# bexcite/ptudes-lab

Hardware: AMD Instinct MI355X
Metric: lidar scans/sec (ICP+EKF) on 128x1024 sweeps (higher is better)
Workload: dtype f64

## Files before the change

### ptudes-lab_amd/csrc/icp_kernels.h

```cpp
#pragma once
#include "devmath.h"
#include "diag.h"
#include <stdint.h>
#include <type_traits>

#define EMPTY_KEY 0xFFFFFFFFFFFFFFFFull
#define TOMB_KEY 0xFFFFFFFFFFFFFFFEull
#define KEY_OFF (1 << 20)

#define ERR_KEY_RANGE 1
#define ERR_POOL 2
#define ERR_TABLE 4
#define ERR_VDS_TABLE 8
#define ERR_GN_TIMEOUT 16

struct TabEnt {
    unsigned long long key;
    int blk;
    int head;
};
#define BLK_ID_MASK 0x00FFFFFF

struct VdsEnt {
    unsigned long long key;
    unsigned vmin;
    unsigned pad;
};
struct ScanStats {
    double sigma, err_dt, err_drot;
    int iterations, n_corr_last;
    long long n_in, n_valid, n_down, n_src, sum_cand, map_voxels, map_points;
};

struct DevState {
    int n_in, n_valid, n_down, n_src;
    unsigned gn_epoch;
    int gn_iters, gn_ncorr;
    int gn_abort;
    int dbg_dead_wg;
    long long gn_cand;
    double gn_max_dist, gn_kernel;
    double T_icp[16];
    double lin_sums[32];
    long long gn_phase_clk[8];
    long long seq_clk[8];
    int n_poses, has_ext_guess;
    double pose_first[16], pose_prev[16], pose_last[16];
    double guess[16], new_pose[16];
    double xi[6];
    int do_deskew, pad1;
    double sigma, sse;
    long long n_samples;
    double model_dev[16];
    int prev_n_in, pending_finish;
    int pro_next;
    int n_src_last;
    int n_down_ins;
    int stats_pending;
    int pool_hw, pool_hw_s;
    int free_top, n_live;
    int free_top_s, mig_n;
    int ulist_n, ulist_pad;
    long long map_points;
    unsigned tab_used;
    int err_flags;
    unsigned long long exec_cnt[8];
    unsigned long long sched_cnt[4];
    unsigned long long empty_cnt;
    unsigned long long full_cnt;
    const double* dk_knots;
    const long long* dk_nknots;
    const int* dk_kovf;
    const double* dk_t0t1;
    int* dk_modes;
    int dk_n, dk_pad;
};
#define DK_MODE_NONE 0
#define DK_MODE_CV 1
#define DK_MODE_IMU 2

struct Ctx {
    double max_range, min_range, vs, vds1, vds2, init_thr, min_motion, conv;
    int P, deskew, max_iter, W;
    const float* in_f32;
    const double* in_f64;
// ... 207 lines not shown
            Rt d = rt_mul(rt_inv(rt_from16(sp[0])), rt_from16(sp[2]));
            moved = sqrt(d.t[0] * d.t[0] + d.t[1] * d.t[1] + d.t[2] * d.t[2]) > 5.0 * c.min_motion;
        }
        s_moved = moved ? 1 : 0;
    }
    if (threadIdx.x == 128) {
        Rt dev = rt_from16(sp[4]);
        const double theta = rot_angle(dev.R);
        s_err = sqrt(dev.t[0] * dev.t[0] + dev.t[1] * dev.t[1] + dev.t[2] * dev.t[2]) + 2.0 * c.max_range * sin(0.5 * theta);
    }
    if (threadIdx.x == 192 && !c.ext_guess) {
        Rt last = rt_from16(sp[2]);
        Rt pred = (n_poses >= 2) ? rt_mul(rt_inv(rt_from16(sp[1])), last) : rt_identity();
        Rt lp = (n_poses >= 1) ? last : rt_identity();
        rt_to16(rt_mul(lp, pred), st->guess);
    }
    __syncthreads();
    if (threadIdx.x == 0) {
        double sigma = c.init_thr;
        if (s_moved) {
            const double err = s_err;
            if (err > c.min_motion) { st->sse += err * err; st->n_samples += 1; }
            sigma = (st->n_samples < 1) ? c.init_thr : sqrt(st->sse / (double)st->n_samples);
        }
        st->sigma = sigma;
        st->gn_max_dist = 3.0 * sigma;
        st->gn_kernel = sigma / 3.0;
    }
    __threadfence_block();
    if (s_closed && threadIdx.x < 48) {
        const int a = threadIdx.x >> 4, k = threadIdx.x & 15;
        double* dst = a == 0 ? st->pose_first : a == 1 ? st->pose_prev : st->pose_last;
        if (a > 0 || s_closed == 2) dst[k] = sp[a][k];
    }
    __syncthreads();
    gn_ll_clear_on_wrap(c);
    if (IMU && st->dk_knots) {
        d_imu_coltab(st, c.coltab, c.W, (c.deskew && c.t01 == nullptr) ? 1 : 0, n_poses);
        return;
    }
    if (st->do_deskew && c.t01 == nullptr) {
        double xi[6];
        for (int k = 0; k < 6; ++k) xi[k] = st->xi[k];
        for (int j = threadIdx.x; j < c.W; j += blockDim.x) {
            const double sft = (double)j * (1.0 / (double)c.W) - 0.5;
            double x[6];
            for (int k = 0; k < 6; ++k) x[k] = sft * xi[k];
            const Rt M = se3_exp(x);
            double* o = c.coltab + (size_t)j;
            for (int k = 0; k < 9; ++k) o[(size_t)k * c.W] = M.R[k];
            for (int k = 0; k < 3; ++k) o[(size_t)(9 + k) * c.W] = M.t[k];
        }
    }
}

__global__ __launch_bounds__(256) void k_build_lut(int H, int W, const double* alt_deg, const double* az_deg, double n_mm,
                                                   const double* T16_mm, double* dir_out, double* off_out) {
    const int i = blockIdx.x * 256 + threadIdx.x;
    if (i >= H * W) return;
    const int u = i / W, v = i % W;
    const double kPi = 3.14159265358979323846;
    const double enc = 2.0 * kPi * (1.0 - (double)v / (double)W);
    const double az = -az_deg[u] * kPi / 180.0, phi = alt_deg[u] * kPi / 180.0;
    const double dx = cos(enc + az) * cos(phi), dy = sin(enc + az) * cos(phi), dz = sin(phi);
    const double ox = n_mm * (cos(enc) - dx), oy = n_mm * (sin(enc) - dy), oz = -n_mm * dz;
    const double* T = T16_mm;
    for (int r = 0; r < 3; ++r) {
        dir_out[3 * (size_t)i + r] = (T[4 * r] * dx + T[4 * r + 1] * dy + T[4 * r + 2] * dz) * 1e-3;
        off_out[3 * (size_t)i + r] = (T[4 * r] * ox + T[4 * r + 1] * oy + T[4 * r + 2] * oz + T[4 * r + 3]) * 1e-3;
    }
}

struct Slice { int b, nb, clk; };
__device__ __forceinline__ Slice launch_slice() { Slice s; s.b = (int)blockIdx.x; s.nb = (int)gridDim.x; s.clk = 0; return s; }
#define STAGE_MAX_WAVES 16
#define STAGE_MAX_U 16

struct VdsPass {
    int* slot;
    VdsEnt* tab;
    unsigned mask;
    int* bcnt;
    const double* in;
    double* out;
    int DevState::*n_out;
    int n;
    DevState* st;
};
__device__ __forceinline__ VdsPass vds_pass1(const Ctx& c) { return VdsPass{c.slot1, c.vtab1, c.vmask, c.bcnt1, c.pts, c.fd, &DevState::n_down, c.n_in, c.st}; }
__device__ __forceinline__ VdsPass vds_pass2(const Ctx& c) { return VdsPass{c.slot2, c.vtab2, c.vmask2, c.bcnt2, c.fd, c.src0, &DevState::n_src, c.st->n_down, c.st}; }

template <int U>
__device__ __forceinline__ void vds_claim_u(VdsEnt* tab, unsigned mask, const unsigned long long (&key)[U], const bool (&want)[U],
                                            int (&slot)[U]) {
    unsigned sp[U];
    unsigned long long old[U];
    bool pend[U];
#pragma unroll
    for (int u = 0; u < U; ++u) {
        sp[u] = brick_slot(key[u], mask);
        slot[u] = -1;
        old[u] = key[u];
        if (want[u]) old[u] = atomicCAS(&tab[sp[u]].key, EMPTY_KEY, key[u]);
    }
#pragma unroll
    for (int u = 0; u < U; ++u) {
        pend[u] = want[u] && !(old[u] == EMPTY_KEY || old[u] == key[u]);
        if (want[u] && !pend[u]) slot[u] = (int)sp[u];
    }
    for (unsigned probe = 1; probe <= mask; ++probe) {
        bool anyp = false;
#pragma unroll
        for (int u = 0; u < U; ++u) anyp = anyp || pend[u];
        if (!anyp) break;
#pragma unroll
        for (int u = 0; u < U; ++u)
            if (pend[u]) { sp[u] = (sp[u] + 1) & mask; old[u] = atomicCAS(&tab[sp[u]].key, EMPTY_KEY, key[u]); }
#pragma unroll
        for (int u = 0; u < U; ++u)
            if (pend[u] && (old[u] == EMPTY_KEY || old[u] == key[u])) { slot[u] = (int)sp[u]; pend[u] = false; }
    }
}
template <int U>
__device__ __forceinline__ void vds_bid_u(VdsEnt* tab, const int (&slot)[U], const bool (&want)[U], const int (&idx)[U], int* err_flags) {
#pragma unroll
    for (int u = 0; u < U; ++u) {
        if (!want[u]) continue;
        if (slot[u] < 0) atomicOr(err_flags, ERR_VDS_TABLE);
        else atomicMin(&tab[slot[u]].vmin, (unsigned)idx[u]);
    }
}
struct VdsNoLap { __device__ __forceinline__ void operator()() const {} };
template <int U, class Between = VdsNoLap>
__device__ __forceinline__ void vds_claim_run_heads(VdsEnt* tab, unsigned mask, const unsigned long long (&key)[U], const bool (&has_key)[U],
                                                    const int (&idx)[U], int (&slot_out)[U], unsigned long long* exec_counter, int* err_flags,
                                                    Between between = Between()) {
    const int lane = threadIdx.x & 63;
    bool head[U];
    int slot[U];
#pragma unroll
    for (int u = 0; u < U; ++u) {
        const unsigned long long prev = __shfl_up(key[u], 1);
        const bool prev_has_key = __shfl_up(has_key[u] ? 1 : 0, 1) != 0;
        head[u] = has_key[u] && (lane == 0 || !prev_has_key || prev != key[u]);
    }
    vds_claim_u<U>(tab, mask, key, head, slot);
    {
        int nh = 0;
#pragma unroll
        for (int u = 0; u < U; ++u) nh += __popcll(__ballot(head[u]));
        if (lane == 0 && nh) atomicAdd(exec_counter, (unsigned long long)nh);
    }
    between();
    vds_bid_u<U>(tab, slot, head, idx, err_flags);
#pragma unroll
    for (int u = 0; u < U; ++u) slot_out[u] = head[u] ? slot[u] : -1;
}
template <int U>
__device__ __forceinline__ int block_count_u(const bool (&f)[U]) {
    __shared__ int cnt[STAGE_MAX_WAVES];
    int mine = 0;
#pragma unroll
    for (int u = 0; u < U; ++u) mine += __popcll(__ballot(f[u]));
    if ((threadIdx.x & 63) == 0) cnt[threadIdx.x >> 6] = mine;
    __syncthreads();
    int tot = 0;
    for (int k = 0; k < ((int)blockDim.x >> 6); ++k) tot += cnt[k];
    __syncthreads();
    return tot;
}

template <int U> struct RawF32 { float v[U][3]; };
template <int U>
__device__ __forceinline__ RawF32<U> k1_load_raw(const Ctx& c, const Slice sl) {
    RawF32<U> r;
    const int BS = (int)blockDim.x, base = sl.b * BS * U + (int)threadIdx.x;
#pragma unroll
    for (int u = 0; u < U; ++u) {
        const int i = base + u * BS;
        const bool in = i < c.n_in;
        r.v[u][0] = in ? c.in_f32[3 * (size_t)i] : 0.0f; r.v[u][1] = in ? c.in_f32[3 * (size_t)i + 1] : 0.0f; r.v[u][2] = in ? c.in_f32[3 * (size_t)i + 2] : 0.0f;
    }
    return r;
}
template <int U>
__device__ __forceinline__ void d_deskew_vds1(const Ctx& c, const Slice sl, const RawF32<U>* pre = nullptr, int* wave_valid = nullptr) {
    const int BS = (int)blockDim.x, base = sl.b * BS * U + (int)threadIdx.x;
    DevState* st = c.st;
    DiagLap<diag::stages, false, true> k1(sl.clk != 0 && threadIdx.x == 0);
    const int do_deskew = st->do_deskew;
    int idx[U];
    bool valid[U], keyed[U];
    unsigned long long key[U];
    V3 p[U];
#pragma unroll
    for (int u = 0; u < U; ++u) idx[u] = base + u * BS;
    k1.lap(c, D_k1_entry);
#pragma unroll
    for (int u = 0; u < U; ++u) {
        const int i = idx[u];
        p[u] = v3(0.0, 0.0, 0.0);
        if (i < c.n_in) {
            if (c.in_range) {
                unsigned rg = c.in_range[i];
                if (c.row_mask && !c.row_mask[i / c.W]) rg = 0;
                const double r = (double)rg;
                const double* d = c.lut_dir + 3 * (size_t)i;
                const double* o = c.lut_off + 3 * (size_t)i;
                p[u] = rg ? v3(r * d[0] + o[0], r * d[1] + o[1], r * d[2] + o[2]) : v3(0.0, 0.0, 0.0);
            } else if (c.in_f32) {
                if (pre) p[u] = v3((double)pre->v[u][0], (double)pre->v[u][1], (double)pre->v[u][2]);
                else p[u] = v3((double)c.in_f32[3 * (size_t)i], (double)c.in_f32[3 * (size_t)i + 1], (double)c.in_f32[3 * (size_t)i + 2]);
            } else {
                p[u] = v3(c.in_f64[3 * (size_t)i], c.in_f64[3 * (size_t)i + 1], c.in_f64[3 * (size_t)i + 2]);
            }
        }
    }
    Rt Mcol[2];
    const bool col_period2 = U > 2 && ((2 * BS) % c.W) == 0;
#pragma unroll
    for (int u = 0; u < U; ++u) {
        const int i = idx[u];
        valid[u] = false; keyed[u] = false; key[u] = EMPTY_KEY;
        if (i < c.n_in) {
            if (do_deskew) {
                if (c.t01) {
                    const double s = c.t01[i] - 0.5;
                    double x[6];
                    for (int k = 0; k < 6; ++k) x[k] = s * st->xi[k];
                    p[u] = rt_apply(se3_exp(x), p[u]);
                } else {
                    Rt& M = (u & 1) ? Mcol[1] : Mcol[0];
                    if (u < 2 || !col_period2) {
                        const double* m = c.coltab + (size_t)(i % c.W);
                        for (int k = 0; k < 9; ++k) M.R[k] = m[(size_t)k * c.W];
                        for (int k = 0; k < 3; ++k) M.t[k] = m[(size_t)(9 + k) * c.W];
                    }
                    p[u] = rt_apply(M, p[u]);
                }
            }
            const double r = sqrt(p[u].x * p[u].x + p[u].y * p[u].y + p[u].z * p[u].z);
            valid[u] = (r < c.max_range) && (r > c.min_range);
            if (valid[u]) {
                c.pts[3 * (size_t)i] = p[u].x; c.pts[3 * (size_t)i + 1] = p[u].y; c.pts[3 * (size_t)i + 2] = p[u].z;
                int kx, ky, kz;
                keyed[u] = vox_key(p[u], c.vds1, key[u], kx, ky, kz);
                if (!keyed[u]) atomicOr(&st->err_flags, ERR_KEY_RANGE);
            }
        }
    }
    k1.lap(c, D_k1_load_deskew_store);
    {
        const VdsPass p1 = vds_pass1(c);
        int slot[U];
        vds_claim_run_heads<U>(p1.tab, p1.mask, key, keyed, idx, slot, &st->exec_cnt[4], &st->err_flags, [&] { k1.lap(c, D_k1_claim); });
        k1.lap(c, D_k1_bid);
#pragma unroll
        for (int u = 0; u < U; ++u)
            if (idx[u] < p1.n) p1.slot[idx[u]] = slot[u];
    }
    k1.lap(c, D_k1_slot1);
    if (wave_valid) {
        int nvw = 0;
#pragma unroll
        for (int u = 0; u < U; ++u) nvw += __popcll(__ballot(valid[u]));
        *wave_valid += nvw;
    } else {
        const int nv = block_count_u<U>(valid);
        if (threadIdx.x == 0 && nv) atomicAdd(&st->n_valid, nv);
    }
    k1.lap(c, D_k1_count);
}

template <int U> struct PreI32 { int v[U]; };
template <int U>
__device__ __forceinline__ PreI32<U> stage_load_i32(const int* arr, int n, const Slice sl) {
    PreI32<U> r;
    const int BS = (int)blockDim.x, base = sl.b * BS * U + (int)threadIdx.x;
#pragma unroll
    for (int u = 0; u < U; ++u) { const int i = base + u * BS; r.v[u] = (i < n) ? arr[i] : -1; }
    return r;
}

__device__ __forceinline__ int block_offset_part(const int* bcnt, int b) {
    int s = 0;
    for (int k = threadIdx.x; k < b; k += (int)blockDim.x) s += bcnt[k];
    return s;
}
__device__ __forceinline__ int block_offset(int s) {
    __shared__ int red[STAGE_MAX_WAVES];
    const int nw = (int)blockDim.x >> 6;
    for (int o = 32; o > 0; o >>= 1) s += __shfl_down(s, o);
    if ((threadIdx.x & 63) == 0) red[threadIdx.x >> 6] = s;
    __syncthreads();
    int tot = 0;
    for (int k = 0; k < nw; ++k) tot += red[k];
    __syncthreads();
    return tot;
}
template <int U>
__device__ __forceinline__ void block_rank_u(const bool (&f)[U], int (&rk)[U], int& total) {
    __shared__ int red[STAGE_MAX_U][STAGE_MAX_WAVES];
    const int lane = threadIdx.x & 63, wv = threadIdx.x >> 6, nw = (int)blockDim.x >> 6;
    int within[U];
#pragma unroll
    for (int u = 0; u < U; ++u) {
        const unsigned long long m = __ballot(f[u]);
        within[u] = __popcll(m & ((1ull << lane) - 1ull));
        if (lane == 0) red[u][wv] = __popcll(m);
    }
    __syncthreads();
    int running = 0;
#pragma unroll
    for (int u = 0; u < U; ++u) {
        int off = 0, tot = 0;
        for (int k = 0; k < nw; ++k) { const int v = red[u][k]; if (k < wv) off += v; tot += v; }
        rk[u] = running + off + within[u];
        running += tot;
    }
    total = running;
    __syncthreads();
}
#define LOOKBACK_POLLS (1u << 22)
__device__ __forceinline__ void lookback_publish(int* bcnt, int b, unsigned tag, int count) {
    if (threadIdx.x == 0) __hip_atomic_store(&bcnt[b], (int)((tag << 16) | (unsigned)count), __ATOMIC_RELAXED, __HIP_MEMORY_SCOPE_AGENT);
}
__device__ __forceinline__ int lookback_offset(const int* bcnt, int b, unsigned tag, DevState* st) {
    int s = 0;
    bool bad = false;
    for (int k = threadIdx.x; k < b; k += (int)blockDim.x) {
        unsigned polls = 0;
        for (;;) {
            const unsigned v = (unsigned)__hip_atomic_load(&bcnt[k], __ATOMIC_RELAXED, __HIP_MEMORY_SCOPE_AGENT);
            if ((v >> 16) == tag) { s += (int)(v & 0xFFFFu); break; }
            if (++polls > LOOKBACK_POLLS || ((polls & 1023u) == 0u && __hip_atomic_load(&st->gn_abort, __ATOMIC_RELAXED, __HIP_MEMORY_SCOPE_AGENT) != 0)) { bad = true; break; }
            __builtin_amdgcn_s_sleep(1);
        }
    }
    if (bad) { atomicOr(&st->err_flags, ERR_GN_TIMEOUT); __hip_atomic_store(&st->gn_abort, 1, __ATOMIC_RELAXED, __HIP_MEMORY_SCOPE_AGENT); }
    return block_offset(s);
}
__device__ __forceinline__ unsigned lookback_tag(int scan_k) { return ((unsigned)scan_k % 0xFFFFu) + 1u; }
static_assert(STAGE_MAX_U * 1024 < (1 << 16), "the look-back word keeps a block's count in 16 bits");

template <int U>
__device__ __forceinline__ void d_count_winners(const VdsPass& p, const Slice sl) {
    const int BS = (int)blockDim.x, base = sl.b * BS * U + (int)threadIdx.x;
    int idx[U], s[U];
    bool w[U];
#pragma unroll
    for (int u = 0; u < U; ++u) { idx[u] = base + u * BS; s[u] = (idx[u] < p.n) ? p.slot[idx[u]] : -1; }
    {
        unsigned vm[U];
#pragma unroll
        for (int u = 0; u < U; ++u) vm[u] = (s[u] >= 0) ? p.tab[s[u]].vmin : 0u;
#pragma unroll
        for (int u = 0; u < U; ++u) w[u] = (s[u] >= 0) && (vm[u] == (unsigned)idx[u]);
    }
    const int nw = block_count_u<U>(w);
    if (threadIdx.x == 0) p.bcnt[sl.b] = nw;
}

template <int U, bool LB>
__device__ __forceinline__ void d_compact_winners(const VdsPass& p, const Slice sl, const PreI32<U>* pre = nullptr, unsigned tag = 0u) {
    const int BS = (int)blockDim.x, base = sl.b * BS * U + (int)threadIdx.x;
    int idx[U], s[U], rk[U];
    bool w[U];
    int off_part = 0;
    if (!LB) off_part = block_offset_part(p.bcnt, sl.b);
#pragma unroll
    for (int u = 0; u < U; ++u) { idx[u] = base + u * BS; s[u] = pre ? pre->v[u] : ((idx[u] < p.n) ? p.slot[idx[u]] : -1); }
    {
        unsigned vm[U];
#pragma unroll
        for (int u = 0; u < U; ++u) vm[u] = (s[u] >= 0) ? p.tab[s[u]].vmin : 0u;
#pragma unroll
        for (int u = 0; u < U; ++u) w[u] = (s[u] >= 0) && (vm[u] == (unsigned)idx[u]);
    }
    double q[U][3];
#pragma unroll
    for (int u = 0; u < U; ++u) {
        const size_t i = (size_t)idx[u];
        if (w[u]) { q[u][0] = p.in[3 * i]; q[u][1] = p.in[3 * i + 1]; q[u][2] = p.in[3 * i + 2]; }
    }
    int total;
    block_rank_u<U>(w, rk, total);
    int off;
    if (LB) {
        lookback_publish(p.bcnt, sl.b, tag, total);
        off = lookback_offset(p.bcnt, sl.b, tag, p.st);
    } else {
        off = block_offset(off_part);
    }
#pragma unroll
    for (int u = 0; u < U; ++u) {
        if (!w[u]) continue;
        const size_t o = (size_t)(off + rk[u]) * 3;
        p.out[o] = q[u][0]; p.out[o + 1] = q[u][1]; p.out[o + 2] = q[u][2];
        p.tab[s[u]].key = EMPTY_KEY;
        p.tab[s[u]].vmin = 0xFFFFFFFFu;
    }
    if (threadIdx.x == 0 && sl.b == sl.nb - 1) p.st->*p.n_out = off + total;
}

template <int U>
__device__ __forceinline__ void d_vds2_fd(const Ctx& c, const Slice sl) {
    const int BS = (int)blockDim.x, base = sl.b * BS * U + (int)threadIdx.x;
    const VdsPass p2 = vds_pass2(c);
    int idx[U];
    bool act[U];
    unsigned long long key[U];
#pragma unroll
    for (int u = 0; u < U; ++u) { idx[u] = base + u * BS; act[u] = idx[u] < p2.n; key[u] = EMPTY_KEY; }
    {
        double q[U][3];
#pragma unroll
        for (int u = 0; u < U; ++u) {
            const size_t j = (size_t)idx[u];
            q[u][0] = q[u][1] = q[u][2] = 0.0;
            if (act[u]) { q[u][0] = p2.in[3 * j]; q[u][1] = p2.in[3 * j + 1]; q[u][2] = p2.in[3 * j + 2]; }
        }
#pragma unroll
        for (int u = 0; u < U; ++u) {
            if (!act[u]) continue;
            int kx, ky, kz;
            vox_key(v3(q[u][0], q[u][1], q[u][2]), c.vds2, key[u], kx, ky, kz);
        }
    }
    int slot[U];
    vds_claim_run_heads<U>(p2.tab, p2.mask, key, act, idx, slot, &c.st->exec_cnt[5], &c.st->err_flags);
#pragma unroll
    for (int u = 0; u < U; ++u)
        if (act[u]) p2.slot[idx[u]] = slot[u];
}

template <class CT>
__device__ __forceinline__ int map_find(const CT& c, unsigned long long key) {
    unsigned s = brick_slot(key, c.tmask);
    for (unsigned probe = 0; probe <= c.tmask; ++probe) {
        const TabEnt e = c.tab[s];
        if (e.key == key) return e.blk;
        if (e.key == EMPTY_KEY) return -1;
        s = (s + 1) & c.tmask;
    }
    return -1;
}

__device__ __forceinline__ double sqrt_gate(double M) {
    if (!(M > 0.0) || !(M < 1.0e150)) return (M > 0.0) ? M : 0.0;
    double T = M * M;
    for (int k = 0; k < 64 && sqrt(__longlong_as_double(__double_as_longlong(T) - 1)) >= M; ++k)
        T = __longlong_as_double(__double_as_longlong(T) - 1);
    for (int k = 0; k < 64 && sqrt(T) < M; ++k) T = __longlong_as_double(__double_as_longlong(T) + 1);
    return T;
}

template <int CTRL>
__device__ __forceinline__ double dpp_f64(double v) {
    const unsigned long long u = (unsigned long long)__double_as_longlong(v);
    const unsigned lo = (unsigned)__builtin_amdgcn_update_dpp(0, (int)(unsigned)u, CTRL, 0xF, 0xF, true);
    const unsigned hi = (unsigned)__builtin_amdgcn_update_dpp(0, (int)(unsigned)(u >> 32), CTRL, 0xF, 0xF, true);
    return __longlong_as_double((long long)(((unsigned long long)hi << 32) | lo));
}
__device__ __forceinline__ double group_min32(double v) {
    v = fmin(v, dpp_f64<0xB1>(v));
    v = fmin(v, dpp_f64<0x4E>(v));
    v = fmin(v, dpp_f64<0x141>(v));
    v = fmin(v, dpp_f64<0x140>(v));
    return fmin(v, __shfl_xor(v, 16));
}
__device__ __forceinline__ unsigned group_min32(unsigned v) {
    v = min(v, (unsigned)__builtin_amdgcn_update_dpp(0, (int)v, 0xB1, 0xF, 0xF, true));
    v = min(v, (unsigned)__builtin_amdgcn_update_dpp(0, (int)v, 0x4E, 0xF, 0xF, true));
    v = min(v, (unsigned)__builtin_amdgcn_update_dpp(0, (int)v, 0x141, 0xF, 0xF, true));
    v = min(v, (unsigned)__builtin_amdgcn_update_dpp(0, (int)v, 0x140, 0xF, 0xF, true));
    return min(v, (unsigned)__shfl_xor((int)v, 16));
}

__device__ __forceinline__ int group_sum32(int v) {
    v += __builtin_amdgcn_update_dpp(0, v, 0xB1, 0xF, 0xF, true);
    v += __builtin_amdgcn_update_dpp(0, v, 0x4E, 0xF, 0xF, true);
    v += __builtin_amdgcn_update_dpp(0, v, 0x141, 0xF, 0xF, true);
    v += __builtin_amdgcn_update_dpp(0, v, 0x140, 0xF, 0xF, true);
// ... 1751 lines not shown
    const int cnt = blk_hdr(c, b)[0];
    if (cnt <= 0) return;
    const int o = atomicAdd(counter, cnt);
    const double* X = blk_x(c, b);
    for (int j = 0; j < cnt; ++j) {
        if (o + j >= max_points) break;
        out[3 * (size_t)(o + j)] = X[3 * j]; out[3 * (size_t)(o + j) + 1] = X[3 * j + 1]; out[3 * (size_t)(o + j) + 2] = X[3 * j + 2];
    }
}

__global__ __launch_bounds__(256) void k_deskew_only(Ctx c, const double* xyz, const double* t01, int n, double* out) {
    const int i = blockIdx.x * 256 + threadIdx.x;
    if (i >= n) return;
    const DevState* st = c.st;
    V3 p = v3(xyz[3 * (size_t)i], xyz[3 * (size_t)i + 1], xyz[3 * (size_t)i + 2]);
    if (c.deskew && st->n_poses >= 2) {
        double xi[6], x[6];
        se3_log(rt_mul(rt_inv(rt_from16(st->pose_prev)), rt_from16(st->pose_last)), xi);
        const double sft = t01[i] - 0.5;
        for (int k = 0; k < 6; ++k) x[k] = sft * xi[k];
        p = rt_apply(se3_exp(x), p);
    }
    out[3 * (size_t)i] = p.x; out[3 * (size_t)i + 1] = p.y; out[3 * (size_t)i + 2] = p.z;
}

__global__ __launch_bounds__(1024) void k_range_stats(const unsigned* range, int H, int W, const unsigned char* row_mask,
                                                      double to_m, double* out) {
    __shared__ double sh[1024];
    __shared__ double shmin[1024], shmax[1024];
    __shared__ double s_mean, s_n;
    const int tid = threadIdx.x, n_all = H * W;
    for (int pass = 0; pass < 2; ++pass) {
        const double mean = pass ? s_mean : 0.0;
        double acc = 0.0, cnt = 0.0, lo = 1.7976931348623157e308, hi = -1.7976931348623157e308;
        for (int i = tid; i < n_all; i += 1024) {
            const unsigned r = range[i];
            if (r == 0 || (row_mask && !row_mask[i / W])) continue;
            const double x = (double)r * to_m;
            if (pass == 0) { acc += x; cnt += 1.0; lo = fmin(lo, x); hi = fmax(hi, x); }
            else { const double d = x - mean; acc += d * d; }
        }
        sh[tid] = acc;
        __syncthreads();
        for (int o = 512; o > 0; o >>= 1) { if (tid < o) sh[tid] += sh[tid + o]; __syncthreads(); }
        const double total = sh[0];
        __syncthreads();
        if (pass == 0) {
            sh[tid] = cnt; shmin[tid] = lo; shmax[tid] = hi;
            __syncthreads();
            for (int o = 512; o > 0; o >>= 1) {
                if (tid < o) { sh[tid] += sh[tid + o]; shmin[tid] = fmin(shmin[tid], shmin[tid + o]); shmax[tid] = fmax(shmax[tid], shmax[tid + o]); }
                __syncthreads();
            }
            if (tid == 0) {
                s_n = sh[0];
                s_mean = sh[0] > 0.0 ? total / sh[0] : 0.0;
                out[0] = sh[0]; out[1] = s_mean; out[3] = shmin[0]; out[4] = shmax[0];
            }
            __syncthreads();
        } else if (tid == 0) {
            out[2] = s_n > 0.0 ? total / s_n : 0.0;
        }
    }
}

struct EkfState;
struct SeqCtx {
    Ctx c;
    const float* scan_base;
    long long scan_stride_floats;
    int input_is_range, n_scans;
    double* fd_buf[2];
    EkfState* ekf;
    const double* imu;
    const int* imu_end;
    double *res_poses, *res_t, *rows;
};
__device__ __forceinline__ Ctx load_seq_ctx(const SeqCtx* a, int s, int scan_k) {
    Ctx c = a[s].c;
    c.fd = a[s].fd_buf[scan_k & 1];
    const float* p = a[s].scan_base + (size_t)scan_k * (size_t)a[s].scan_stride_floats;
    if (a[s].input_is_range) { c.in_range = (const unsigned*)p; c.in_f32 = nullptr; }
    else { c.in_f32 = p; c.in_range = nullptr; }
    c.in_f32 = uniform_ptr(c.in_f32); c.in_range = uniform_ptr(c.in_range);
    c.pts = uniform_ptr(c.pts);
    c.slot1 = uniform_ptr(c.slot1); c.vtab1 = uniform_ptr(c.vtab1); c.bcnt1 = uniform_ptr(c.bcnt1);
    c.slot2 = uniform_ptr(c.slot2); c.vtab2 = uniform_ptr(c.vtab2); c.bcnt2 = uniform_ptr(c.bcnt2);
    c.fd = uniform_ptr(c.fd); c.fdw = uniform_ptr(c.fdw); c.src0 = uniform_ptr(c.src0); c.coltab = uniform_ptr(c.coltab);
    c.pslot = uniform_ptr(c.pslot); c.nxt = uniform_ptr(c.nxt); c.prank = uniform_ptr(c.prank); c.plen = uniform_ptr(c.plen);
    c.tab = uniform_ptr(c.tab); c.blocks = uniform_ptr(c.blocks); c.free_stack = uniform_ptr(c.free_stack); c.st = uniform_ptr(c.st);
    c.bhdr = uniform_ptr(c.bhdr); c.bfirst = uniform_ptr(c.bfirst); c.big_base = uniform_ptr(c.big_base);
    c.free_stack_s = uniform_ptr(c.free_stack_s); c.mig_list = uniform_ptr(c.mig_list);
    return c;
}
__global__ __launch_bounds__(1024) void k_scan_prologue(Ctx c) { d_scan_prologue<false>(c); }
__global__ __launch_bounds__(1024) void k_scan_prologue_imu(Ctx c) { d_scan_prologue<true>(c); }
__global__ __launch_bounds__(1024) void kb_scan_prologue(const SeqCtx* a, int scan_k) {
    const Ctx c = load_seq_ctx(a, blockIdx.y, scan_k);
    d_scan_prologue<false>(c);
}
__global__ __launch_bounds__(1024) void kb_scan_prologue_imu(const SeqCtx* a, int scan_k) {
    const Ctx c = load_seq_ctx(a, blockIdx.y, scan_k);
    d_scan_prologue<true>(c);
}
__global__ __launch_bounds__(256) void k_deskew_vds1(Ctx c) { d_deskew_vds1<1>(c, launch_slice()); }
__global__ __launch_bounds__(256) void kb_deskew_vds1(const SeqCtx* a, int scan_k) {
    const Ctx c = load_seq_ctx(a, blockIdx.y, scan_k);
    d_deskew_vds1<1>(c, launch_slice());
}
__global__ __launch_bounds__(256) void k_count_w1(Ctx c) { d_count_winners<1>(vds_pass1(c), launch_slice()); }
__global__ __launch_bounds__(256) void kb_count_w1(const SeqCtx* a, int scan_k) {
    const Ctx c = load_seq_ctx(a, blockIdx.y, scan_k);
    d_count_winners<1>(vds_pass1(c), launch_slice());
}
__global__ __launch_bounds__(256) void k_compact_fd(Ctx c) { d_compact_winners<1, false>(vds_pass1(c), launch_slice()); }
__global__ __launch_bounds__(256) void kb_compact_fd(const SeqCtx* a, int scan_k) {
    const Ctx c = load_seq_ctx(a, blockIdx.y, scan_k);
    d_compact_winners<1, false>(vds_pass1(c), launch_slice());
}
__global__ __launch_bounds__(256) void k_vds2_fd(Ctx c) { d_vds2_fd<1>(c, launch_slice()); }
__global__ __launch_bounds__(256) void kb_vds2_fd(const SeqCtx* a, int scan_k) {
    const Ctx c = load_seq_ctx(a, blockIdx.y, scan_k);
    d_vds2_fd<1>(c, launch_slice());
}
__global__ __launch_bounds__(256) void k_count_w2(Ctx c) { d_count_winners<1>(vds_pass2(c), launch_slice()); }
__global__ __launch_bounds__(256) void kb_count_w2(const SeqCtx* a, int scan_k) {
    const Ctx c = load_seq_ctx(a, blockIdx.y, scan_k);
    d_count_winners<1>(vds_pass2(c), launch_slice());
}
__global__ __launch_bounds__(256) void k_compact_src(Ctx c) { d_compact_winners<1, false>(vds_pass2(c), launch_slice()); }
__global__ __launch_bounds__(256) void kb_compact_src(const SeqCtx* a, int scan_k) {
    const Ctx c = load_seq_ctx(a, blockIdx.y, scan_k);
    d_compact_winners<1, false>(vds_pass2(c), launch_slice());
}
__global__ __launch_bounds__(256) void k_map_insert_a(Ctx c, const double* pts_in, const int* n_ptr, int n_fixed, int use_pose) { d_map_insert_a<1>(c, pts_in, n_ptr, n_fixed, use_pose, launch_slice()); }
__global__ __launch_bounds__(256) void kb_map_insert_a(const SeqCtx* a, int scan_k) {
    const Ctx c = load_seq_ctx(a, blockIdx.y, scan_k);
    d_map_insert_a<1>(c, c.fd, &c.st->n_down_ins, 0, 1, launch_slice());
}
__global__ __launch_bounds__(256) void k_map_insert_b(Ctx c, const int* n_ptr, int n_fixed) { d_map_insert_b<1>(c, n_ptr, n_fixed, launch_slice()); }
__global__ __launch_bounds__(256) void kb_map_insert_b(const SeqCtx* a, int scan_k) {
    const Ctx c = load_seq_ctx(a, blockIdx.y, scan_k);
    d_map_insert_b<1>(c, &c.st->n_down_ins, 0, launch_slice());
}
__global__ __launch_bounds__(256) void k_map_insert_c(Ctx c, const int* n_ptr, int n_fixed) { d_map_insert_c<1>(c, n_ptr, n_fixed, launch_slice()); }
__global__ __launch_bounds__(256) void kb_map_insert_c(const SeqCtx* a, int scan_k) {
    const Ctx c = load_seq_ctx(a, blockIdx.y, scan_k);
    d_map_insert_c<1>(c, &c.st->n_down_ins, 0, launch_slice());
}
__global__ __launch_bounds__(256) void k_map_prune(Ctx c, const double* origin_xyz, int use_new_pose) { d_map_prune<1>(c, origin_xyz, use_new_pose, launch_slice()); }
__global__ __launch_bounds__(256) void kb_map_prune(const SeqCtx* a, int scan_k) {
    const Ctx c = load_seq_ctx(a, blockIdx.y, scan_k);
    d_map_prune<1>(c, nullptr, 1, launch_slice());
}
__global__ __launch_bounds__(256) void k_map_rebuild(Ctx c) { d_map_rebuild(c, launch_slice()); }
__global__ __launch_bounds__(256) void kb_map_rebuild(const SeqCtx* a, int scan_k) {
    const Ctx c = load_seq_ctx(a, blockIdx.y, scan_k);
    d_map_rebuild(c, launch_slice());
}

#define GN_MAX_SEQ 256
__device__ __forceinline__ bool kx_assign(int S, int& s, int& G, int& wg) {
    const int x = (int)(blockIdx.x & 7u), j = (int)(blockIdx.x >> 3), J = (int)(gridDim.x >> 3);
    const int spx = S <= 8 ? 1 : (S <= 16 ? 2 : 4);
    G = J / spx;
    s = x + 8 * (j / G);
    wg = j % G;
    return s < S;
}
template <int PC, int GC>
__global__ __launch_bounds__(GN8_MAX_THREADS) SEQ_OCC void kx_gn_loop8(const SeqCtx* a, int S, int scan_k) {
    int s, G, wg;
    if (!kx_assign(S, s, G, wg)) return;
    const Ctx c = load_seq_ctx(a, s, scan_k);
    gn8_body<PC, GC>(c, 0, G, wg);
}
template <int PC>
__global__ __launch_bounds__(GN_MAX_THREADS) void kx_gn_loop(const SeqCtx* a, int S, int scan_k) {
    int s, G, wg;
    if (!kx_assign(S, s, G, wg)) return;
    const Ctx c = load_seq_ctx(a, s, scan_k);
    gn_loop_body<PC, true, true>(c, 0, G, wg);
}
```

### ptudes-lab_amd/csrc/seq_kernel.h

```cpp
#pragma once
#include "ekf_kernels.h"
#include "icp_kernels.h"

#define TEAM_BAR_POLLS (1u << 23)
__device__ __forceinline__ bool team_sync(unsigned* word, unsigned n, unsigned& target, int* abort_word, DevState* st, const bool local) {
    __shared__ int s_bad;
    if (n <= 1u) {
        asm volatile("s_waitcnt vmcnt(0)" ::: "memory");
        __syncthreads();
        __builtin_amdgcn_fence(__ATOMIC_ACQUIRE, "agent");
        return true;
    }
    if (local) asm volatile("s_waitcnt vmcnt(0)" ::: "memory");
    __syncthreads();
    target += n;
    if (threadIdx.x == 0) {
        int bad = 0;
        if (!local) __builtin_amdgcn_fence(__ATOMIC_RELEASE, "agent");
        __hip_atomic_fetch_add(word, 1u, __ATOMIC_RELAXED, __HIP_MEMORY_SCOPE_AGENT);
        unsigned polls = 0;
        while (__hip_atomic_load(word, __ATOMIC_RELAXED, __HIP_MEMORY_SCOPE_AGENT) < target) {
            __builtin_amdgcn_s_sleep(2);
            if ((++polls & 255u) == 0u && (gn_abort_seen(abort_word) || polls > TEAM_BAR_POLLS)) { bad = 1; break; }
        }
        if (bad) {
            if (st) gn_raise_abort(st);
            __hip_atomic_store(abort_word, 1, __ATOMIC_RELAXED, __HIP_MEMORY_SCOPE_AGENT);
        }
        s_bad = bad;
    }
    __syncthreads();
    __builtin_amdgcn_fence(__ATOMIC_ACQUIRE, "agent");
    return s_bad == 0;
}
struct TeamEnv { unsigned* word; int* abort_word; DevState* st; bool local; };
__device__ __forceinline__ bool team_sync(const TeamEnv& e, unsigned n, unsigned& target) { return team_sync(e.word, n, target, e.abort_word, e.st, e.local); }
__device__ __forceinline__ unsigned xcc_id() {
    unsigned v;
    asm volatile("s_getreg_b32 %0, hwreg(HW_REG_XCC_ID)" : "=s"(v));
    return v & 0xFu;
}

#define SEQ_FAIL 0xFFFFFFFFu
#ifndef SEQ_U
#define SEQ_U 8
#endif
#ifndef SEQ_UM
#define SEQ_UM SEQ_U
#endif
#ifndef SEQ_UM_ALT
#define SEQ_UM_ALT 4
#endif
#ifndef SEQ_U2
#define SEQ_U2 16
#endif
__device__ __noinline__ void sq_prologue(const SeqCtx* a, int s, int k) { d_scan_prologue(load_seq_ctx(a, s, k), true); }
__device__ __noinline__ unsigned sq_prepare(const SeqCtx* a, int s, int k, int wg, int nw, unsigned target, unsigned* word, bool local) {
    const Ctx c = load_seq_ctx(a, s, k);
    DevState* st = c.st;
    const int BS = (int)blockDim.x * SEQ_U, nbs = (c.n_in + BS - 1) / BS;
    const int BS2 = (int)blockDim.x * SEQ_U2, nbs2 = (c.n_in + BS2 - 1) / BS2;
    Slice sl;
    sl.nb = nbs; sl.clk = wg == 0 ? 1 : 0;
    const TeamEnv te = {word, &st->gn_abort, st, local};
    DiagLap<diag::stages, false, false> sq(wg == 0 && threadIdx.x == 0);
    if (wg == 0 && st->pro_next != k + 1) sq_prologue(a, s, k);
    sq.lap(c, D_sq_prologue);
    if (!team_sync(te, (unsigned)nw, target)) return SEQ_FAIL;
    sq.lap(c, D_sq_wait_prologue);
    int wave_valid = 0;
    if (c.in_f32 && !c.in_range) {
        RawF32<SEQ_U> raw;
        sl.b = wg;
        if (wg < nbs) raw = k1_load_raw<SEQ_U>(c, sl);
        for (sl.b = wg; sl.b < nbs; sl.b += nw) {
            const RawF32<SEQ_U> cur = raw;
            Slice nx = sl;
            nx.b = sl.b + nw;
            if (nx.b < nbs) raw = k1_load_raw<SEQ_U>(c, nx);
            d_deskew_vds1<SEQ_U>(c, sl, &cur, &wave_valid);
        }
    } else {
        for (sl.b = wg; sl.b < nbs; sl.b += nw) d_deskew_vds1<SEQ_U>(c, sl, nullptr, &wave_valid);
    }
    if ((threadIdx.x & 63) == 0 && wave_valid) atomicAdd(&st->n_valid, wave_valid);
    sq.lap(c, D_sq_deskew_vds1);
    if (!team_sync(te, (unsigned)nw, target)) return SEQ_FAIL;
    sq.lap(c, D_sq_wait_deskew_vds1);
    sl.nb = nbs2;
    const unsigned tag = lookback_tag(k);
    {
        PreI32<SEQ_U2> pw;
        sl.b = wg;
        if (wg < nbs2) pw = stage_load_i32<SEQ_U2>(c.slot1, c.n_in, sl);
        for (sl.b = wg; sl.b < nbs2; sl.b += nw) {
            const PreI32<SEQ_U2> cur = pw;
            Slice nx = sl;
            nx.b = sl.b + nw;
            if (nx.b < nbs2) pw = stage_load_i32<SEQ_U2>(c.slot1, c.n_in, nx);
            d_compact_winners<SEQ_U2, true>(vds_pass1(c), sl, &cur, tag);
        }
    }
    sq.lap(c, D_sq_compact_fd);
    if (!team_sync(te, (unsigned)nw, target)) return SEQ_FAIL;
    sq.lap(c, D_sq_wait_compact_fd);
    const int nbf = (st->n_down + BS2 - 1) / BS2;
    sl.nb = nbf;
    for (sl.b = wg; sl.b < nbf; sl.b += nw) d_vds2_fd<SEQ_U2>(c, sl);
    sq.lap(c, D_sq_vds2);
    if (!team_sync(te, (unsigned)nw, target)) return SEQ_FAIL;
    sq.lap(c, D_sq_wait_vds2);
    for (sl.b = wg; sl.b < nbf; sl.b += nw) d_compact_winners<SEQ_U2, true>(vds_pass2(c), sl, nullptr, tag);
    sq.lap(c, D_sq_compact_src);
    return target;
}
__device__ __forceinline__ int sq_grab(unsigned* ctr) {
    __shared__ int s_blk;
    __syncthreads();
    if (threadIdx.x == 0) s_blk = (int)__hip_atomic_fetch_add(ctr, 1u, __ATOMIC_RELAXED, __HIP_MEMORY_SCOPE_AGENT);
    __syncthreads();
    return s_blk;
}
template <int UM>
__device__ __noinline__ unsigned sq_map_update(const SeqCtx* a, int s, int k, int wg, int nw, unsigned target, int rebuild, unsigned* word, unsigned* ctr, bool local) {
    const Ctx c = load_seq_ctx(a, s, k);
    DevState* st = c.st;
    const int BS = (int)blockDim.x, BU = BS * UM, nbd = (st->n_down_ins + BU - 1) / BU;
    Slice sl;
    sl.nb = nbd; sl.clk = 0;
    const TeamEnv te = {word, &st->gn_abort, st, local};
    DiagLap<diag::stages, false, false> sq(wg == 0 && threadIdx.x == 0);
    for (sl.b = sq_grab(ctr); sl.b < nbd; sl.b = sq_grab(ctr)) d_map_insert_a<UM, true>(c, c.fd, &st->n_down_ins, 0, 1, sl);
    sq.lap(c, D_sq_insert_a);
    if (!team_sync(te, (unsigned)nw, target)) return SEQ_FAIL;
    sq.lap(c, D_sq_wait_insert_a);
    const int nbl = (st->ulist_n + BU - 1) / BU;
    sl.nb = nbl;
    for (sl.b = sq_grab(ctr + 1); sl.b < nbl; sl.b = sq_grab(ctr + 1)) d_map_insert_b<UM, true, true>(c, &st->ulist_n, 0, sl);
    sq.lap(c, D_sq_insert_b);
    if (!team_sync(te, (unsigned)nw, target)) return SEQ_FAIL;
    if (wg == 0 && threadIdx.x == 0) st->ulist_n = 0;
    sq.lap(c, D_sq_wait_insert_b);
    const int nvb = blk_virtual_count(c, st);
    const int nbpu = (nvb + BU - 1) / BU;
    sl.nb = nbpu;
    for (sl.b = sq_grab(ctr + 3); sl.b < nbpu; sl.b = sq_grab(ctr + 3)) d_map_prune<UM, true>(c, nullptr, 1, sl);
    sq.lap(c, D_sq_prune);
    if (c.n_small > 0) {
        if (!team_sync(te, (unsigned)nw, target)) return SEQ_FAIL;
        const int nm = st->mig_n < c.n_small ? st->mig_n : c.n_small, nbm = (nm + BS - 1) / BS;
        sl.nb = nbm;
        for (sl.b = sq_grab(ctr + 2); sl.b < nbm; sl.b = sq_grab(ctr + 2)) d_map_migrate(c, sl);
        if (!team_sync(te, (unsigned)nw, target)) return SEQ_FAIL;
        if (wg == 0 && threadIdx.x == 0) st->mig_n = 0;
    }
    const int nbp = (blk_virtual_count(c, st) + BS - 1) / BS;
    sl.nb = nbp;
    if (rebuild) {
        if (!team_sync(te, (unsigned)nw, target)) return SEQ_FAIL;
        unsigned long long* tw = (unsigned long long*)c.tab;
        const size_t nwords = ((size_t)c.tmask + 1) * (sizeof(TabEnt) / 8);
        for (size_t i = (size_t)wg * BS + threadIdx.x; i < nwords; i += (size_t)nw * BS) tw[i] = ~0ull;
        if (wg == 0 && threadIdx.x == 0) st->tab_used = 0u;
        if (!team_sync(te, (unsigned)nw, target)) return SEQ_FAIL;
        for (sl.b = sq_grab(ctr + 4); sl.b < nbp; sl.b = sq_grab(ctr + 4)) d_map_rebuild(c, sl);
    }
    return target;
}
template <int PC, int GC>
__device__ __noinline__ void sq_gauss_newton(const SeqCtx* a, int s, int k, int G, int wg) {
    const Ctx c = load_seq_ctx(a, s, k);
    gn8_body<PC, GC>(c, 0, G, wg);
}
__device__ __noinline__ void sq_filter(const SeqCtx* a, int s, int k) {
    const SeqCtx* my = a + s;
    const int i0 = my->imu_end[k], i1 = (k + 1 < my->n_scans) ? my->imu_end[k + 1] : i0;
    d_ekf_step(my->ekf, my->imu, i0, i1, my->c.traj + 16 * (size_t)k, nullptr, my->res_poses + 16 * (size_t)k,
               my->res_t + k, my->rows + 8 * (size_t)k, 1);
    if (k + 1 < my->n_scans) {
        __syncthreads();
        const Ctx c = load_seq_ctx(a, s, k + 1);
        d_scan_prologue(c, true);
        __syncthreads();
        if (threadIdx.x == 0) c.st->pro_next = k + 2;
    }
}

struct SeqRun {
    int S, k0, k1, with_ekf, rebuild_every, G;
    int um_alt;
    int force_agent;
    int dbg_dead_block;
    int dbg_dead_round;
    int balance_margin;
};
// ... 211 lines not shown
```

Baseline: 43360.

## Recompute deskewed points in compaction instead of storing full pts array

```diff
diff --git a/ptudes-lab_amd/csrc/col_pair.h b/ptudes-lab_amd/csrc/col_pair.h
--- /dev/null
+++ b/ptudes-lab_amd/csrc/col_pair.h
@@ -0,0 +1,8 @@
+#pragma once
+#if defined(__HIPCC__)
+#define COL_PAIR_FN __host__ __device__ inline
+#else
+#define COL_PAIR_FN inline
+#endif
+COL_PAIR_FN bool col_pair_fixed(int bs, int U, int W) { return W > 0 && U >= 2 && ((bs * U) % W) == 0 && ((2 * bs) % W) == 0; }
+COL_PAIR_FN int col_pair_column(int bs, int W, int tid, int odd) { return (tid + (odd ? bs : 0)) % W; }
diff --git a/ptudes-lab_amd/csrc/icp_kernels.h b/ptudes-lab_amd/csrc/icp_kernels.h
--- a/ptudes-lab_amd/csrc/icp_kernels.h
+++ b/ptudes-lab_amd/csrc/icp_kernels.h
@@ -1,6 +1,7 @@
 #pragma once
 #include "devmath.h"
 #include "diag.h"
+#include "col_pair.h"
 #include <stdint.h>
 #include <type_traits>
 
@@ -374,13 +375,72 @@
     unsigned mask;
     int* bcnt;
     const double* in;
+    const Ctx* raw;
     double* out;
     int DevState::*n_out;
     int n;
     DevState* st;
 };
-__device__ __forceinline__ VdsPass vds_pass1(const Ctx& c) { return VdsPass{c.slot1, c.vtab1, c.vmask, c.bcnt1, c.pts, c.fd, &DevState::n_down, c.n_in, c.st}; }
-__device__ __forceinline__ VdsPass vds_pass2(const Ctx& c) { return VdsPass{c.slot2, c.vtab2, c.vmask2, c.bcnt2, c.fd, c.src0, &DevState::n_src, c.st->n_down, c.st}; }
+__device__ __forceinline__ VdsPass vds_pass1(const Ctx& c) { return VdsPass{c.slot1, c.vtab1, c.vmask, c.bcnt1, nullptr, &c, c.fd, &DevState::n_down, c.n_in, c.st}; }
+__device__ __forceinline__ VdsPass vds_pass2(const Ctx& c) { return VdsPass{c.slot2, c.vtab2, c.vmask2, c.bcnt2, c.fd, nullptr, c.src0, &DevState::n_src, c.st->n_down, c.st}; }
+
+struct RawPt { unsigned w[6]; };
+__device__ __forceinline__ RawPt raw_of_v3(const V3 p) {
+    RawPt r;
+    r.w[0] = (unsigned)__double2loint(p.x); r.w[1] = (unsigned)__double2hiint(p.x);
+    r.w[2] = (unsigned)__double2loint(p.y); r.w[3] = (unsigned)__double2hiint(p.y);
+    r.w[4] = (unsigned)__double2loint(p.z); r.w[5] = (unsigned)__double2hiint(p.z);
+    return r;
+}
+__device__ __forceinline__ RawPt raw_of_f64(const double* a, size_t i) { return raw_of_v3(v3(a[3 * i], a[3 * i + 1], a[3 * i + 2])); }
+__device__ __forceinline__ V3 raw_as_f64(const RawPt& r) {
+    return v3(__hiloint2double((int)r.w[1], (int)r.w[0]), __hiloint2double((int)r.w[3], (int)r.w[2]), __hiloint2double((int)r.w[5], (int)r.w[4]));
+}
+__device__ __forceinline__ RawPt raw_of_f32(float x, float y, float z) {
+    RawPt r;
+    r.w[0] = __float_as_uint(x); r.w[1] = __float_as_uint(y); r.w[2] = __float_as_uint(z); r.w[3] = r.w[4] = r.w[5] = 0u;
+    return r;
+}
+__device__ __forceinline__ RawPt raw_request(const Ctx& c, int i) {
+    if (c.in_range) { RawPt r; r.w[0] = c.in_range[i]; r.w[1] = r.w[2] = r.w[3] = r.w[4] = r.w[5] = 0u; return r; }
+    if (c.in_f32) return raw_of_f32(c.in_f32[3 * (size_t)i], c.in_f32[3 * (size_t)i + 1], c.in_f32[3 * (size_t)i + 2]);
+    return raw_of_f64(c.in_f64, (size_t)i);
+}
+__device__ __forceinline__ V3 raw_sensor(const Ctx& c, int i, const RawPt& r) {
+    if (c.in_range) {
+        unsigned rg = r.w[0];
+        if (c.row_mask && !c.row_mask[i / c.W]) rg = 0;
+        const double rd = (double)rg;
+        const double* d = c.lut_dir + 3 * (size_t)i;
+        const double* o = c.lut_off + 3 * (size_t)i;
+        return rg ? v3(rd * d[0] + o[0], rd * d[1] + o[1], rd * d[2] + o[2]) : v3(0.0, 0.0, 0.0);
+    }
+    if (c.in_f32) return v3((double)__uint_as_float(r.w[0]), (double)__uint_as_float(r.w[1]), (double)__uint_as_float(r.w[2]));
+    return raw_as_f64(r);
+}
+__device__ __forceinline__ Rt coltab_load(const Ctx& c, int col) {
+    Rt M;
+    const double* m = c.coltab + (size_t)col;
+    for (int k = 0; k < 9; ++k) M.R[k] = m[(size_t)k * c.W];
+    for (int k = 0; k < 3; ++k) M.t[k] = m[(size_t)(9 + k) * c.W];
+    return M;
+}
+__device__ __forceinline__ V3 deskew_t01(const Ctx& c, int i, const V3 p) {
+    const double s = c.t01[i] - 0.5;
+    double x[6];
+    for (int k = 0; k < 6; ++k) x[k] = s * c.st->xi[k];
+    return rt_apply(se3_exp(x), p);
+}
+__device__ __forceinline__ V3 deskew_apply(const Ctx& c, int i, const V3 p, const Rt& M) { return c.t01 ? deskew_t01(c, i, p) : rt_apply(M, p); }
+__device__ __forceinline__ V3 deskew_apply(const Ctx& c, int i, const V3 p) { return c.t01 ? deskew_t01(c, i, p) : rt_apply(coltab_load(c, i % c.W), p); }
+__device__ __forceinline__ V3 deskewed_point(const Ctx& c, int i, const RawPt& r, int do_deskew, const Rt& M) {
+    const V3 p = raw_sensor(c, i, r);
+    return do_deskew ? deskew_apply(c, i, p, M) : p;
+}
+__device__ __forceinline__ V3 deskewed_point(const Ctx& c, int i, const RawPt& r, int do_deskew) {
+    const V3 p = raw_sensor(c, i, r);
+    return do_deskew ? deskew_apply(c, i, p) : p;
+}
 
 template <int U>
 __device__ __forceinline__ void vds_claim_u(VdsEnt* tab, unsigned mask, const unsigned long long (&key)[U], const bool (&want)[U],
@@ -475,8 +535,16 @@
     }
     return r;
 }
-template <int U>
-__device__ __forceinline__ void d_deskew_vds1(const Ctx& c, const Slice sl, const RawF32<U>* pre = nullptr, int* wave_valid = nullptr) {
+struct ColPair { Rt M[2]; };
+__device__ __forceinline__ ColPair col_pair_load(const Ctx& c) {
+    ColPair cp;
+    cp.M[0] = coltab_load(c, col_pair_column((int)blockDim.x, c.W, (int)threadIdx.x, 0));
+    cp.M[1] = coltab_load(c, col_pair_column((int)blockDim.x, c.W, (int)threadIdx.x, 1));
+    return cp;
+}
+template <int U, bool PAIR = false>
+__device__ __forceinline__ void d_deskew_vds1(const Ctx& c, const Slice sl, const RawF32<U>* pre = nullptr, int* wave_valid = nullptr,
+                                              const ColPair* hoist = nullptr) {
     const int BS = (int)blockDim.x, base = sl.b * BS * U + (int)threadIdx.x;
     DevState* st = c.st;
     DiagLap<diag::stages, false, true> k1(sl.clk != 0 && threadIdx.x == 0);
@@ -492,21 +560,7 @@
     for (int u = 0; u < U; ++u) {
         const int i = idx[u];
         p[u] = v3(0.0, 0.0, 0.0);
-        if (i < c.n_in) {
-            if (c.in_range) {
-                unsigned rg = c.in_range[i];
-                if (c.row_mask && !c.row_mask[i / c.W]) rg = 0;
-                const double r = (double)rg;
-                const double* d = c.lut_dir + 3 * (size_t)i;
-                const double* o = c.lut_off + 3 * (size_t)i;
-                p[u] = rg ? v3(r * d[0] + o[0], r * d[1] + o[1], r * d[2] + o[2]) : v3(0.0, 0.0, 0.0);
-            } else if (c.in_f32) {
-                if (pre) p[u] = v3((double)pre->v[u][0], (double)pre->v[u][1], (double)pre->v[u][2]);
-                else p[u] = v3((double)c.in_f32[3 * (size_t)i], (double)c.in_f32[3 * (size_t)i + 1], (double)c.in_f32[3 * (size_t)i + 2]);
-            } else {
-                p[u] = v3(c.in_f64[3 * (size_t)i], c.in_f64[3 * (size_t)i + 1], c.in_f64[3 * (size_t)i + 2]);
-            }
-        }
+        if (i < c.n_in) p[u] = raw_sensor(c, i, (pre && c.in_f32 && !c.in_range) ? raw_of_f32(pre->v[u][0], pre->v[u][1], pre->v[u][2]) : raw_request(c, i));
     }
     Rt Mcol[2];
     const bool col_period2 = U > 2 && ((2 * BS) % c.W) == 0;
@@ -516,25 +570,13 @@
         valid[u] = false; keyed[u] = false; key[u] = EMPTY_KEY;
         if (i < c.n_in) {
             if (do_deskew) {
-                if (c.t01) {
-                    const double s = c.t01[i] - 0.5;
-                    double x[6];
-                    for (int k = 0; k < 6; ++k) x[k] = s * st->xi[k];
-                    p[u] = rt_apply(se3_exp(x), p[u]);
-                } else {
-                    Rt& M = (u & 1) ? Mcol[1] : Mcol[0];
-                    if (u < 2 || !col_period2) {
-                        const double* m = c.coltab + (size_t)(i % c.W);
-                        for (int k = 0; k < 9; ++k) M.R[k] = m[(size_t)k * c.W];
-                        for (int k = 0; k < 3; ++k) M.t[k] = m[(size_t)(9 + k) * c.W];
-                    }
-                    p[u] = rt_apply(M, p[u]);
-                }
+                Rt& M = (u & 1) ? Mcol[1] : Mcol[0];
+                if (!PAIR && !c.t01 && (u < 2 || !col_period2)) M = coltab_load(c, i % c.W);
+                p[u] = PAIR ? deskew_apply(c, i, p[u], hoist->M[u & 1]) : deskew_apply(c, i, p[u], M);
             }
             const double r = sqrt(p[u].x * p[u].x + p[u].y * p[u].y + p[u].z * p[u].z);
             valid[u] = (r < c.max_range) && (r > c.min_range);
             if (valid[u]) {
-                c.pts[3 * (size_t)i] = p[u].x; c.pts[3 * (size_t)i + 1] = p[u].y; c.pts[3 * (size_t)i + 2] = p[u].z;
                 int kx, ky, kz;
                 keyed[u] = vox_key(p[u], c.vds1, key[u], kx, ky, kz);
                 if (!keyed[u]) atomicOr(&st->err_flags, ERR_KEY_RANGE);
@@ -653,8 +695,9 @@
     if (threadIdx.x == 0) p.bcnt[sl.b] = nw;
 }
 
-template <int U, bool LB>
-__device__ __forceinline__ void d_compact_winners(const VdsPass& p, const Slice sl, const PreI32<U>* pre = nullptr, unsigned tag = 0u) {
+template <int U, bool LB, bool RAW, bool PAIR = false>
+__device__ __forceinline__ void d_compact_winners(const VdsPass& p, const Slice sl, const PreI32<U>* pre = nullptr, unsigned tag = 0u,
+                                                  const ColPair* hoist = nullptr) {
     const int BS = (int)blockDim.x, base = sl.b * BS * U + (int)threadIdx.x;
     int idx[U], s[U], rk[U];
     bool w[U];
@@ -669,12 +712,15 @@
 #pragma unroll
         for (int u = 0; u < U; ++u) w[u] = (s[u] >= 0) && (vm[u] == (unsigned)idx[u]);
     }
-    double q[U][3];
+    RawPt q[U];
+    double qs[U][3];
 #pragma unroll
     for (int u = 0; u < U; ++u) {
-        const size_t i = (size_t)idx[u];
-        if (w[u]) { q[u][0] = p.in[3 * i]; q[u][1] = p.in[3 * i + 1]; q[u][2] = p.in[3 * i + 2]; }
-    }
+        if (!w[u]) continue;
+        if constexpr (RAW) q[u] = raw_request(*p.raw, idx[u]);
+        else { const size_t i = (size_t)idx[u]; qs[u][0] = p.in[3 * i]; qs[u][1] = p.in[3 * i + 1]; qs[u][2] = p.in[3 * i + 2]; }
+    }
+    const int do_deskew = RAW ? p.st->do_deskew : 0;
     int total;
     block_rank_u<U>(w, rk, total);
     int off;
@@ -684,13 +730,30 @@
     } else {
         off = block_offset(off_part);
     }
-#pragma unroll
-    for (int u = 0; u < U; ++u) {
-        if (!w[u]) continue;
-        const size_t o = (size_t)(off + rk[u]) * 3;
-        p.out[o] = q[u][0]; p.out[o + 1] = q[u][1]; p.out[o + 2] = q[u][2];
-        p.tab[s[u]].key = EMPTY_KEY;
-        p.tab[s[u]].vmin = 0xFFFFFFFFu;
+    constexpr int CH = U < 4 ? U : 4;
+#pragma unroll
+    for (int u0 = 0; u0 < U; u0 += CH) {
+        double vx[CH], vy[CH], vz[CH];
+#pragma unroll
+        for (int j = 0; j < CH; ++j) {
+            const int u = u0 + j;
+            V3 v = v3(0.0, 0.0, 0.0);
+            if (w[u]) {
+                if (!RAW) v = v3(qs[u][0], qs[u][1], qs[u][2]);
+                else if (PAIR) v = deskewed_point(*p.raw, idx[u], q[u], do_deskew, hoist->M[u & 1]);
+                else v = deskewed_point(*p.raw, idx[u], q[u], do_deskew);
+            }
+            vx[j] = v.x; vy[j] = v.y; vz[j] = v.z;
+        }
+#pragma unroll
+        for (int j = 0; j < CH; ++j) {
+            const int u = u0 + j;
+            if (!w[u]) continue;
+            const size_t o = (size_t)(off + rk[u]) * 3;
+            p.out[o] = vx[j]; p.out[o + 1] = vy[j]; p.out[o + 2] = vz[j];
+            p.tab[s[u]].key = EMPTY_KEY;
+            p.tab[s[u]].vmin = 0xFFFFFFFFu;
+        }
     }
     if (threadIdx.x == 0 && sl.b == sl.nb - 1) p.st->*p.n_out = off + total;
 }
@@ -2608,6 +2671,7 @@
     const float* p = a[s].scan_base + (size_t)scan_k * (size_t)a[s].scan_stride_floats;
     if (a[s].input_is_range) { c.in_range = (const unsigned*)p; c.in_f32 = nullptr; }
     else { c.in_f32 = p; c.in_range = nullptr; }
+    c.in_f64 = nullptr; c.t01 = nullptr;
     c.in_f32 = uniform_ptr(c.in_f32); c.in_range = uniform_ptr(c.in_range);
     c.pts = uniform_ptr(c.pts);
     c.slot1 = uniform_ptr(c.slot1); c.vtab1 = uniform_ptr(c.vtab1); c.bcnt1 = uniform_ptr(c.bcnt1);
@@ -2639,10 +2703,10 @@
     const Ctx c = load_seq_ctx(a, blockIdx.y, scan_k);
     d_count_winners<1>(vds_pass1(c), launch_slice());
 }
-__global__ __launch_bounds__(256) void k_compact_fd(Ctx c) { d_compact_winners<1, false>(vds_pass1(c), launch_slice()); }
+__global__ __launch_bounds__(256) void k_compact_fd(Ctx c) { d_compact_winners<1, false, true>(vds_pass1(c), launch_slice()); }
 __global__ __launch_bounds__(256) void kb_compact_fd(const SeqCtx* a, int scan_k) {
     const Ctx c = load_seq_ctx(a, blockIdx.y, scan_k);
-    d_compact_winners<1, false>(vds_pass1(c), launch_slice());
+    d_compact_winners<1, false, true>(vds_pass1(c), launch_slice());
 }
 __global__ __launch_bounds__(256) void k_vds2_fd(Ctx c) { d_vds2_fd<1>(c, launch_slice()); }
 __global__ __launch_bounds__(256) void kb_vds2_fd(const SeqCtx* a, int scan_k) {
@@ -2654,10 +2718,10 @@
     const Ctx c = load_seq_ctx(a, blockIdx.y, scan_k);
     d_count_winners<1>(vds_pass2(c), launch_slice());
 }
-__global__ __launch_bounds__(256) void k_compact_src(Ctx c) { d_compact_winners<1, false>(vds_pass2(c), launch_slice()); }
+__global__ __launch_bounds__(256) void k_compact_src(Ctx c) { d_compact_winners<1, false, false>(vds_pass2(c), launch_slice()); }
 __global__ __launch_bounds__(256) void kb_compact_src(const SeqCtx* a, int scan_k) {
     const Ctx c = load_seq_ctx(a, blockIdx.y, scan_k);
-    d_compact_winners<1, false>(vds_pass2(c), launch_slice());
+    d_compact_winners<1, false, false>(vds_pass2(c), launch_slice());
 }
 __global__ __launch_bounds__(256) void k_map_insert_a(Ctx c, const double* pts_in, const int* n_ptr, int n_fixed, int use_pose) { d_map_insert_a<1>(c, pts_in, n_ptr, n_fixed, use_pose, launch_slice()); }
 __global__ __launch_bounds__(256) void kb_map_insert_a(const SeqCtx* a, int scan_k) {
diff --git a/ptudes-lab_amd/csrc/seq_kernel.h b/ptudes-lab_amd/csrc/seq_kernel.h
--- a/ptudes-lab_amd/csrc/seq_kernel.h
+++ b/ptudes-lab_amd/csrc/seq_kernel.h
@@ -55,6 +55,40 @@
 #define SEQ_U2 16
 #endif
 __device__ __noinline__ void sq_prologue(const SeqCtx* a, int s, int k) { d_scan_prologue(load_seq_ctx(a, s, k), true); }
+template <bool PAIR>
+__device__ __forceinline__ void sq_k1_blocks(const Ctx& c, Slice sl, int wg, int nw, int nbs, int& wave_valid) {
+    ColPair cp;
+    if (PAIR) cp = col_pair_load(c);
+    if (c.in_f32 && !c.in_range) {
+        RawF32<SEQ_U> raw;
+        sl.b = wg;
+        if (wg < nbs) raw = k1_load_raw<SEQ_U>(c, sl);
+        for (sl.b = wg; sl.b < nbs; sl.b += nw) {
+            const RawF32<SEQ_U> cur = raw;
+            Slice nx = sl;
+            nx.b = sl.b + nw;
+            if (nx.b < nbs) raw = k1_load_raw<SEQ_U>(c, nx);
+            d_deskew_vds1<SEQ_U, PAIR>(c, sl, &cur, &wave_valid, &cp);
+        }
+    } else {
+        for (sl.b = wg; sl.b < nbs; sl.b += nw) d_deskew_vds1<SEQ_U, PAIR>(c, sl, nullptr, &wave_valid, &cp);
+    }
+}
+template <bool PAIR>
+__device__ __forceinline__ void sq_k3_blocks(const Ctx& c, Slice sl, int wg, int nw, int nbs2, unsigned tag) {
+    ColPair cp;
+    if (PAIR) cp = col_pair_load(c);
+    PreI32<SEQ_U2> pw;
+    sl.b = wg;
+    if (wg < nbs2) pw = stage_load_i32<SEQ_U2>(c.slot1, c.n_in, sl);
+    for (sl.b = wg; sl.b < nbs2; sl.b += nw) {
+        const PreI32<SEQ_U2> cur = pw;
+        Slice nx = sl;
+        nx.b = sl.b + nw;
+        if (nx.b < nbs2) pw = stage_load_i32<SEQ_U2>(c.slot1, c.n_in, nx);
+        d_compact_winners<SEQ_U2, true, true, PAIR>(vds_pass1(c), sl, &cur, tag, &cp);
+    }
+}
 __device__ __noinline__ unsigned sq_prepare(const SeqCtx* a, int s, int k, int wg, int nw, unsigned target, unsigned* word, bool local) {
     const Ctx c = load_seq_ctx(a, s, k);
     DevState* st = c.st;
@@ -68,39 +102,18 @@
     sq.lap(c, D_sq_prologue);
     if (!team_sync(te, (unsigned)nw, target)) return SEQ_FAIL;
     sq.lap(c, D_sq_wait_prologue);
+    const bool pair = st->do_deskew && !c.t01 && col_pair_fixed((int)blockDim.x, SEQ_U, c.W) && col_pair_fixed((int)blockDim.x, SEQ_U2, c.W);
     int wave_valid = 0;
-    if (c.in_f32 && !c.in_range) {
-        RawF32<SEQ_U> raw;
-        sl.b = wg;
-        if (wg < nbs) raw = k1_load_raw<SEQ_U>(c, sl);
-        for (sl.b = wg; sl.b < nbs; sl.b += nw) {
-            const RawF32<SEQ_U> cur = raw;
-            Slice nx = sl;
-            nx.b = sl.b + nw;
-            if (nx.b < nbs) raw = k1_load_raw<SEQ_U>(c, nx);
-            d_deskew_vds1<SEQ_U>(c, sl, &cur, &wave_valid);
-        }
-    } else {
-        for (sl.b = wg; sl.b < nbs; sl.b += nw) d_deskew_vds1<SEQ_U>(c, sl, nullptr, &wave_valid);
-    }
+    if (pair) sq_k1_blocks<true>(c, sl, wg, nw, nbs, wave_valid);
+    else sq_k1_blocks<false>(c, sl, wg, nw, nbs, wave_valid);
     if ((threadIdx.x & 63) == 0 && wave_valid) atomicAdd(&st->n_valid, wave_valid);
     sq.lap(c, D_sq_deskew_vds1);
     if (!team_sync(te, (unsigned)nw, target)) return SEQ_FAIL;
     sq.lap(c, D_sq_wait_deskew_vds1);
     sl.nb = nbs2;
     const unsigned tag = lookback_tag(k);
-    {
-        PreI32<SEQ_U2> pw;
-        sl.b = wg;
-        if (wg < nbs2) pw = stage_load_i32<SEQ_U2>(c.slot1, c.n_in, sl);
-        for (sl.b = wg; sl.b < nbs2; sl.b += nw) {
-            const PreI32<SEQ_U2> cur = pw;
-            Slice nx = sl;
-            nx.b = sl.b + nw;
-            if (nx.b < nbs2) pw = stage_load_i32<SEQ_U2>(c.slot1, c.n_in, nx);
-            d_compact_winners<SEQ_U2, true>(vds_pass1(c), sl, &cur, tag);
-        }
-    }
+    if (pair) sq_k3_blocks<true>(c, sl, wg, nw, nbs2, tag);
+    else sq_k3_blocks<false>(c, sl, wg, nw, nbs2, tag);
     sq.lap(c, D_sq_compact_fd);
     if (!team_sync(te, (unsigned)nw, target)) return SEQ_FAIL;
     sq.lap(c, D_sq_wait_compact_fd);
@@ -110,7 +123,7 @@
     sq.lap(c, D_sq_vds2);
     if (!team_sync(te, (unsigned)nw, target)) return SEQ_FAIL;
     sq.lap(c, D_sq_wait_vds2);
-    for (sl.b = wg; sl.b < nbf; sl.b += nw) d_compact_winners<SEQ_U2, true>(vds_pass2(c), sl, nullptr, tag);
+    for (sl.b = wg; sl.b < nbf; sl.b += nw) d_compact_winners<SEQ_U2, true, false>(vds_pass2(c), sl, nullptr, tag);
     sq.lap(c, D_sq_compact_src);
     return target;
 }
```

After: 43760 (median of 6 runs). No clear change (+0.9%).
